# PaddleCV-SIG/MedicalSeg

Hardware: AMD Instinct MI355X
Metric: 3D-voxels/sec fwd+bwd, VNet 128^3 fp32 (higher is better)
Workload: dtype f32

## Files before the change

### medicalseg_amd/csrc/msk_conv_wbf.hip

```cpp
#include <type_traits>
#include "msk_wbf.h"
#ifndef WBF_TIN_SYNC
#define WBF_TIN_SYNC 1
#endif

#ifndef WBF_PROBE
#define WBF_PROBE 0
#endif
typedef _Float16 f16x8 __attribute__((ext_vector_type(8)));
typedef _Float16 f16x2 __attribute__((ext_vector_type(2)));

namespace {

constexpr int nxi_of(int K) { return K == 5 ? 8 : 6; }

__device__ __forceinline__ void split3_one(float x, unsigned short& hi, unsigned short& mid, unsigned short& lo) {
  hi = __builtin_bit_cast(unsigned short, (__bf16)x);
  const float r = x - __uint_as_float((unsigned)hi << 16);
  mid = __builtin_bit_cast(unsigned short, (__bf16)r);
  const float r2 = r - __uint_as_float((unsigned)mid << 16);
  lo = __builtin_bit_cast(unsigned short, (__bf16)r2);
}
__device__ __forceinline__ unsigned pack_f16_pair(float a, float b) {
  f32x2 v = {a, b};
// ... 533 lines not shown
  float4 win[WIN][2];
  const int t0 = blockIdx.z * a.t_per, t1 = min(a.T, t0 + a.t_per);
#pragma unroll
  for (int j = 0; j < WIN; ++j) dy_at(4 * t0 + j - PADW, win[j][0], win[j][1]);
  for (int t = t0; t < t1; ++t) {
#if WBF_TIN_SYNC
    __builtin_amdgcn_s_barrier();
#endif
    float4 nxt[4][2];
#pragma unroll
    for (int j = 0; j < 4; ++j) {
      const int w = 4 * (t + 1) + KEEP - PADW + j;
      if (t + 1 < t1) dy_at(w, nxt[j][0], nxt[j][1]);
      else nxt[j][0] = nxt[j][1] = z4;
    }
    float v[8][8];
    if (WV) {
#pragma unroll
      for (int q = 0; q < 2; ++q) {
        float wx[8], wy[8], wz[8], ww[8];
#pragma unroll
        for (int j = 0; j < 8; ++j) {
          const float4 e = j < WIN ? win[j < WIN ? j : 0][q] : z4;
          wx[j] = e.x; wy[j] = e.y; wz[j] = e.z; ww[j] = e.w;
        }
        tin_transform<0, K>(wx, v[q * 4 + 0]);
        tin_transform<0, K>(wy, v[q * 4 + 1]);
        tin_transform<0, K>(wz, v[q * 4 + 2]);
        tin_transform<0, K>(ww, v[q * 4 + 3]);
      }
#pragma unroll
      for (int xi = 0; xi < NXI; ++xi) store_xi<K, NP>(vb + t * tstep + (long)xi * a.v_xi, plane, v, xi, sc2);
    }
    if (WY) {
#pragma unroll
      for (int q = 0; q < 2; ++q) {
        float wx[8], wy[8], wz[8], ww[8];
#pragma unroll
        for (int j = 0; j < 4; ++j) {
          const float4 e = win[PADW + j][q];
          wx[j] = e.x; wy[j] = e.y; wz[j] = e.z; ww[j] = e.w;
        }
#pragma unroll
        for (int j = 4; j < 8; ++j) wx[j] = wy[j] = wz[j] = ww[j] = 0.f;
        tin_transform<1, K>(wx, v[q * 4 + 0]);
        tin_transform<1, K>(wy, v[q * 4 + 1]);
        tin_transform<1, K>(wz, v[q * 4 + 2]);
        tin_transform<1, K>(ww, v[q * 4 + 3]);
      }
#pragma unroll
      for (int xi = 0; xi < NXI; ++xi) store_xi<K, NP>(yb2 + t * tstep + (long)xi * b.y_xi, plane, v, xi, sc2);
    }
#pragma unroll
    for (int j = 0; j < KEEP; ++j) {
      win[j][0] = win[j + 4][0];
      win[j][1] = win[j + 4][1];
    }
#pragma unroll
    for (int j = 0; j < 4; ++j) {
      win[KEEP + j][0] = nxt[j][0];
      win[KEEP + j][1] = nxt[j][1];
    }
  }
  }
  if (want_cmax) wbf_cmax_commit(b.y_cmax, cg, cmx, true);
}

struct GemmArgs {
  const char* V;
  const char* U;
  float* M;
  int N, T, KC, CN, LD, LH, DP, HP;
  int tiles_d, tiles_h, ngrp, ksplit, kc_per;
  int tpb, nblk;
  long v_xi, v_plane;
  long u_xi;
  long m_xi;
};

__device__ __forceinline__ uint4 buf_load16(__amdgpu_buffer_rsrc_t r, unsigned lane_bytes, unsigned uniform_bytes) {
  return __builtin_bit_cast(uint4, __builtin_amdgcn_raw_buffer_load_b128(r, (int)lane_bytes, (int)uniform_bytes, 0));
}

typedef int i32x4 __attribute__((ext_vector_type(4)));
__device__ __forceinline__ void wbf_dma16(i32x4 rs, unsigned lds_addr, unsigned voff, unsigned soff) {
  asm volatile("s_mov_b32 m0, %0\n\ts_nop 0\n\tbuffer_load_dwordx4 %1, %2, %3 offen lds" ::"s"(lds_addr), "v"(voff), "s"(rs), "s"(soff) : "memory");
}

#define WBF_MFMA(acc, av, bv) \
  acc = __builtin_amdgcn_mfma_f32_32x32x16_bf16(__builtin_bit_cast(bf16x8, av), __builtin_bit_cast(bf16x8, bv), acc, 0, 0, 0)
#define WBF_MFMA_H(acc, av, bv) \
  acc = __builtin_amdgcn_mfma_f32_32x32x16_f16(__builtin_bit_cast(f16x8, av), __builtin_bit_cast(f16x8, bv), acc, 0, 0, 0)

template <int TH>
__device__ __forceinline__ void frag_pos(int r, int& a, int& b) {
  if (TH == 16) {
    if (r < 4) { a = 0; b = r; }
    else if (r < 12) { a = 0; b = r + 4; }
    else if (r < 16) { a = 0; b = r - 8; }
    else if (r < 20) { a = 1; b = r - 4; }
    else if (r < 28) { a = 1; b = r - 16; }
    else { a = 1; b = r - 28; }
  } else if (TH == 8) {
    if (r < 4) { a = 0; b = r; }
    else if (r < 12) { a = 1; b = r - 4; }
    else if (r < 16) { a = 0; b = r - 8; }
    else if (r < 20) { a = 3; b = r - 16; }
    else if (r < 28) { a = 2; b = r - 20; }
    else { a = 3; b = r - 24; }
  } else {
    a = r / TH;
    b = r % TH;
  }
}

template <int MR, int WM, int WN, int TD, int TH, int K, int NP, int BPF = 1>
__global__ void __launch_bounds__(WM * WN * 64)
wbf_gemm_k(GemmArgs a) {
  static_assert((WM * WN == 4 || WM * WN == 2) && WM * MR * 32 == TD * TH, "tile shape");
  constexpr int NT = WM * WN * 64;
  constexpr int NXI = nxi_of(K), T2 = K * K, PADK = (K - 1) / 2;
  constexpr int HDt = TD + K - 1, HPt = TH + K - 1, NSLOT = HDt * HPt, NPL = 2 * NP, NIT = NPL * NSLOT, ROUNDS = (NIT + NT - 1) / NT;
  __shared__ uint4 lds[ROUNDS * NT];

  const int tid = threadIdx.x;
  const int wave = __builtin_amdgcn_readfirstlane(tid >> 6), lane = tid & 63, li = lane & 31, lh = lane >> 5;
  const int wm = wave / WN, wn = wave % WN;

#pragma unroll 1
  for (int rep = 0; rep < a.tpb; ++rep) {
  int b = blockIdx.x + rep * gridDim.x;
  if (b >= a.nblk) break;
  if (rep > 0) __syncthreads();
  const int xi = b % NXI;
  b /= NXI;
  const int grp = b % a.ngrp;
  b /= a.ngrp;
  const int thi = b % a.tiles_h;
  b /= a.tiles_h;
  const int tdi = b % a.tiles_d;
  b /= a.tiles_d;
  const int t = b % a.T;
  b /= a.T;
  const int n = b % a.N;
  const int ks = b / a.N;

  unsigned voff[ROUNDS];
#pragma unroll
  for (int r = 0; r < ROUNDS; ++r) {
    int it = r * NT + tid;
    if (it >= NIT) it = 0;
    const int pk = it / NSLOT, slot = it - pk * NSLOT;
    const int row = slot / HPt, col = slot - row * HPt;
    voff[r] = (unsigned)(pk * a.v_plane + ((long)row * a.HP + col) * 16);
  }
  const char* vtile = a.V + (long)xi * a.v_xi + ((long)(n * a.T + t) * a.KC) * NPL * a.v_plane +
                      ((long)(tdi * TD + 2 - PADK) * a.HP + thi * TH + 2 - PADK) * 16;
  const __amdgpu_buffer_rsrc_t vres = __builtin_amdgcn_make_buffer_rsrc((void*)vtile, 0, 0xFFFFFFF0u, 0x00020000);
  const __amdgpu_buffer_rsrc_t ures =
      __builtin_amdgcn_make_buffer_rsrc((void*)(a.U + (long)xi * a.u_xi), 0, 0xFFFFFFF0u, 0x00020000);
  const unsigned ulane = (unsigned)(lh * a.CN + (grp * WN + wn) * 32 + li) * 16u;
  const unsigned ustep = (unsigned)a.CN * 32u;
  const unsigned uchunk = (unsigned)NP * ustep;
  const unsigned utap = (unsigned)a.KC * uchunk;

  int arow[MR];
#pragma unroll
  for (int mr = 0; mr < MR; ++mr) {
    int fa, fb;
    frag_pos<TH>(li, fa, fb);
// ... 140 lines not shown
  if (xi == 0) { c1 = c2 = c3 = 0.f; return; }
  if (xi == last) { c1 = c2 = 0.f; c3 = 1.f; return; }
  const float sg = (xi & 1) ? 1.f : -1.f;
  const int pr = (xi - 1) >> 1;
  const float p = pr == 0 ? 1.f : (pr == 1 ? 2.f : 0.5f);
  c1 = sg * p;
  c2 = p * p;
  c3 = sg * p * p * p;
}

#ifndef WBF_FUSED_BPF
#define WBF_FUSED_BPF 3
#endif
template <int MR, int WM, int WN, int TD, int TH, int K, int NP, bool STATS, int BPF = (NP == 2 ? WBF_FUSED_BPF : 1), int BL = 0>
__global__ void __launch_bounds__(WM * WN * 64, 2)
wbf_gemm_fused_k(FusedArgs f) {
  static_assert(WM * WN == 4 && WM * MR * 32 == TD * TH, "tile shape");
  const GemmArgs& a = f.g;
  constexpr int NT = WM * WN * 64;
  constexpr int NXI = nxi_of(K), T2 = K * K, PADK = (K - 1) / 2;
  constexpr int HDt = TD + K - 1, HPt = TH + K - 1, NSLOT = HDt * HPt, NPL = 2 * NP, NIT = NPL * NSLOT, ROUNDS = (NIT + NT - 1) / NT;
  constexpr int NBF = T2 * NP;
  constexpr int BROUNDS = (NBF + WM * WN - 1) / (WM * WN);
  static_assert(BL == 0 || NIT % 64 == 0, "weights through LDS: wave-granular tile");
  static_assert(BL != 1 || WN == 1, "B through LDS, whole stage: one column fragment");
  constexpr int PH = WN == 1 ? 4 : 5;
  constexpr int PQ_T[6] = {0, T2 * 1 / PH, T2 * 2 / PH, T2 * 3 / PH, PH > 4 ? T2 * 4 / PH : T2, T2};
  constexpr int PQ_FR = (T2 - PQ_T[PH - 1]) * NP * WN;
  constexpr int PQ_SLOT = PQ_FR * 64;
  static_assert(BL != 2 || (NP == 2 && WM * WN == 4 && WN <= 2 && PQ_T[1] * NP * WN >= 4), "pipelined form: fp16 x 2 pieces, four wavefronts");
  __shared__ uint4 lds[BL == 2 ? 2 * NIT + 2 * PQ_SLOT : (BL ? NIT + NBF * 64 : ROUNDS * NT)];

  const int tid = threadIdx.x;
  const int wave = __builtin_amdgcn_readfirstlane(tid >> 6), lane = tid & 63, li = lane & 31, lh = lane >> 5;
  const int wm = wave / WN, wn = wave % WN;

  int b = (blockIdx.x & 7) * f.per_xcd + (blockIdx.x >> 3);
  if ((int)(blockIdx.x >> 3) >= f.per_xcd || b >= a.nblk) return;
  const int tile_id = b;
  const int thi = b % a.tiles_h;
  b /= a.tiles_h;
  const int tdi = b % a.tiles_d;
  b /= a.tiles_d;
  const int t = b % a.T;
  const int n = b / a.T;

  unsigned voff[ROUNDS];
#pragma unroll
  for (int r = 0; r < ROUNDS; ++r) {
    int it = r * NT + tid;
    if (it >= NIT) it = 0;
    const int pk = it / NSLOT, slot = it - pk * NSLOT;
    const int row = slot / HPt, col = slot - row * HPt;
    voff[r] = (unsigned)(pk * a.v_plane + ((long)row * a.HP + col) * 16);
  }
  const char* vtile0 = a.V + ((long)(n * a.T + t) * a.KC) * NPL * a.v_plane +
                       ((long)(tdi * TD + 2 - PADK) * a.HP + thi * TH + 2 - PADK) * 16;
  const unsigned ulane = (unsigned)(lh * a.CN + wn * 32 + li) * 16u;
  const unsigned ustep = (unsigned)a.CN * 32u;
  const unsigned uchunk = (unsigned)NP * ustep;
  const unsigned utap = (unsigned)a.KC * uchunk;

  int arow[MR];
#pragma unroll
  for (int mr = 0; mr < MR; ++mr) {
    int fa, fb;
    frag_pos<TH>(li, fa, fb);
    arow[mr] = lh * NSLOT + ((wm * MR + mr) * (32 / TH) + fa) * HPt + fb;
  }

  f32x16 yo[4][MR];
#pragma unroll
  for (int i = 0; i < 4; ++i)
#pragma unroll
    for (int mr = 0; mr < MR; ++mr)
#pragma unroll
      for (int j = 0; j < 16; ++j) yo[i][mr][j] = 0.f;

  if constexpr (BL == 2) {
    const unsigned lds0 = (unsigned)(unsigned long)(__attribute__((address_space(3))) void*)lds;
    const int NS = NXI * a.KC;
    const unsigned voff_last = (ROUNDS - 1) * NT + wave * 64 < NIT ? voff[ROUNDS - 1] : voff[ROUNDS - 2];
    const int r_last = (ROUNDS - 1) * NT + wave * 64 < NIT ? ROUNDS - 1 : ROUNDS - 2;
    auto rsrc_of = [](const char* p_) {
      const unsigned long pa = (unsigned long)p_;
      i32x4 r_ = {(int)__builtin_amdgcn_readfirstlane((unsigned)pa), (int)(__builtin_amdgcn_readfirstlane((unsigned)(pa >> 32)) & 0xffffu),
                  (int)0xFFFFFFF0u, 0x00020000};
      return r_;
    };
    auto fill_tile = [&](int s_) {
      const int xi_ = s_ / a.KC, kc_ = s_ - xi_ * a.KC;
      const i32x4 vr = rsrc_of(vtile0 + (long)xi_ * a.v_xi);
      const unsigned so = (unsigned)(kc_ * NPL * a.v_plane);
      const unsigned dst = lds0 + (unsigned)((s_ & 1) * NIT + wave * 64) * 16u;
#pragma unroll
      for (int r = 0; r < ROUNDS - 1; ++r) wbf_dma16(vr, dst + (unsigned)(r * NT) * 16u, voff[r], so);
      wbf_dma16(vr, dst + (unsigned)(r_last * NT) * 16u, voff_last, so);
    };
    auto fill_weights = [&](int s_, auto qc) {
      constexpr int q = decltype(qc)::value;
      constexpr int f0 = PQ_T[q] * NP * WN, nf = (PQ_T[q + 1] - PQ_T[q]) * NP * WN, rounds = (nf + 3) / 4;
      const int xi_ = s_ / a.KC, kc_ = s_ - xi_ * a.KC;
      const i32x4 ur = rsrc_of(a.U + (long)xi_ * a.u_xi);
      const unsigned ukc = (unsigned)kc_ * uchunk;
#pragma unroll
      for (int r = 0; r < rounds; ++r) {
        int fr = r * 4 + wave;
        if (fr >= nf) fr -= 4;
        const int fg = (f0 + fr) / WN, fw = (f0 + fr) % WN;
        wbf_dma16(ur, lds0 + (unsigned)(2 * NIT + ((q + (s_ & PH & 1)) & 1) * PQ_SLOT + fr * 64) * 16u, (unsigned)(lh * a.CN + fw * 32 + li) * 16u,
                  (unsigned)(fg / NP) * utap + ukc + (unsigned)(fg % NP) * ustep);
      }
    };
    f32x16 acc[MR];
    int abase[MR];
    auto run_phase = [&](int s_, auto qc) {
      constexpr int q = decltype(qc)::value;
      constexpr int T0 = PQ_T[q], T1 = PQ_T[q + 1];
      const bool more = s_ + 1 < NS;
      if (q == 1 && more) asm volatile("s_waitcnt vmcnt(%0)" ::"n"(ROUNDS) : "memory");
      else asm volatile("s_waitcnt vmcnt(0)" ::: "memory");
      __builtin_amdgcn_s_barrier();
      asm volatile("" ::: "memory");
      if constexpr (q < PH - 1) fill_weights(s_, std::integral_constant<int, q + 1>{});
      else if (more) fill_weights(s_ + 1, std::integral_constant<int, 0>{});
      if (q == 0 && more) fill_tile(s_ + 1);
      const uint4* bl = lds + 2 * NIT + ((q + (s_ & PH & 1)) & 1) * PQ_SLOT + wn * 64 + lane;
      uint4 aq[2][MR][NP], bq[2][NP];
#pragma unroll
      for (int p = 0; p < NP; ++p) bq[T0 & 1][p] = bl[p * WN * 64];
#pragma unroll
      for (int mr = 0; mr < MR; ++mr) {
        const uint4* ap = lds + abase[mr] + (T0 / K) * HPt + (T0 % K);
#pragma unroll
        for (int p = 0; p < NP; ++p) aq[T0 & 1][mr][p] = ap[p * 2 * NSLOT];
      }
#pragma unroll
      for (int tap = T0; tap < T1; ++tap) {
        const int cur = tap & 1, nx = cur ^ 1;
        if (tap + 1 < T1) {
#pragma unroll
          for (int p = 0; p < NP; ++p) bq[nx][p] = bl[((tap + 1 - T0) * NP + p) * WN * 64];
#pragma unroll
          for (int mr = 0; mr < MR; ++mr) {
            const uint4* ap = lds + abase[mr] + ((tap + 1) / K) * HPt + ((tap + 1) % K);
#pragma unroll
            for (int p = 0; p < NP; ++p) aq[nx][mr][p] = ap[p * 2 * NSLOT];
          }
        }
        __builtin_amdgcn_sched_barrier(0);
        const uint4 bdown = wbf_hi_down(bq[cur][0]);
#pragma unroll
        for (int mr = 0; mr < MR; ++mr) WBF_MFMA_H(acc[mr], aq[cur][mr][NP - 1], bdown);
#pragma unroll
        for (int mr = 0; mr < MR; ++mr) WBF_MFMA_H(acc[mr], aq[cur][mr][0], bq[cur][NP - 1]);
#pragma unroll
        for (int mr = 0; mr < MR; ++mr) WBF_MFMA_H(acc[mr], aq[cur][mr][0], bq[cur][0]);
        __builtin_amdgcn_sched_barrier(0);
      }
    };
    fill_weights(0, std::integral_constant<int, 0>{});
    fill_tile(0);
#pragma unroll 1
    for (int s_ = 0; s_ < NS; ++s_) {
      const int xi = s_ / a.KC, kc = s_ - xi * a.KC;
      if (kc == 0) {
#pragma unroll
        for (int mr = 0; mr < MR; ++mr)
#pragma unroll
          for (int j = 0; j < 16; ++j) acc[mr][j] = 0.f;
      }
#pragma unroll
// ... 1080 lines not shown
```

### medicalseg_amd/csrc/msk_wbf.h

```cpp
#pragma once
#include "msk_conv.h"

typedef __bf16 bf16x8 __attribute__((ext_vector_type(8)));
typedef __bf16 bf16x2 __attribute__((ext_vector_type(2)));
typedef float f32x16 __attribute__((ext_vector_type(16)));
typedef float f32x4 __attribute__((ext_vector_type(4)));
typedef float f32x2 __attribute__((ext_vector_type(2)));

__device__ __forceinline__ void wbf_split3_pair(float x0, float x1, unsigned& hi, unsigned& mid, unsigned& lo) {
  f32x2 x = {x0, x1};
  hi = __builtin_bit_cast(unsigned, __builtin_convertvector(x, bf16x2));
  f32x2 r = {x0 - __uint_as_float(hi << 16), x1 - __uint_as_float(hi & 0xffff0000u)};
  mid = __builtin_bit_cast(unsigned, __builtin_convertvector(r, bf16x2));
  f32x2 r2 = {r.x - __uint_as_float(mid << 16), r.y - __uint_as_float(mid & 0xffff0000u)};
  lo = __builtin_bit_cast(unsigned, __builtin_convertvector(r2, bf16x2));
}

typedef _Float16 wbf_f16x2 __attribute__((ext_vector_type(2)));
__device__ __forceinline__ void wbf_split2h_pair(float x0, float x1, unsigned& hi, unsigned& lo) {
  f32x2 x = {x0, x1};
  const wbf_f16x2 h = __builtin_convertvector(x, wbf_f16x2);
  hi = __builtin_bit_cast(unsigned, h);
  const f32x2 hf = __builtin_convertvector(h, f32x2);
  f32x2 r = {x0 - hf.x, x1 - hf.y};
  lo = __builtin_bit_cast(unsigned, __builtin_convertvector(r, wbf_f16x2));
}
constexpr float kWbfLoScale = 2048.f;
__device__ __forceinline__ void wbf_split2hs_pair(float x0, float x1, unsigned& hi, unsigned& lo) {
  f32x2 x = {x0, x1};
  const wbf_f16x2 h = __builtin_convertvector(x, wbf_f16x2);
  hi = __builtin_bit_cast(unsigned, h);
  const f32x2 hf = __builtin_convertvector(h, f32x2);
  f32x2 r = {(x0 - hf.x) * kWbfLoScale, (x1 - hf.y) * kWbfLoScale};
  lo = __builtin_bit_cast(unsigned, __builtin_convertvector(r, wbf_f16x2));
}
typedef _Float16 wbf_f16x8 __attribute__((ext_vector_type(8)));
__device__ __forceinline__ uint4 wbf_hi_down(uint4 h) {
  const wbf_f16x8 v = __builtin_bit_cast(wbf_f16x8, h) * (_Float16)(1.0f / kWbfLoScale);
  return __builtin_bit_cast(uint4, v);
}
constexpr int kWbfXformHeader = 512;
constexpr int kWbfAmaxWays = 64;
__device__ __forceinline__ float wbf_amax_of(const float* amax) {
  const float4* p = reinterpret_cast<const float4*>(amax);
  float m = 0.f;
#pragma unroll
  for (int i = 0; i < kWbfAmaxWays / 4; ++i) {
    const float4 q = p[i];
    m = fmaxf(fmaxf(m, fmaxf(q.x, q.y)), fmaxf(q.z, q.w));
  }
  return m;
}
__device__ __forceinline__ float wbf_scale_from(float a) {
  if (!(a > 0.f) || !(a < 3.0e38f)) return 1.f;
  int e;
  (void)frexpf(a, &e);
  return ldexpf(1.f, 10 - e);
}
__device__ __forceinline__ float wbf_scale_of(const float* amax) {
  if (!amax) return 1.f;
  return wbf_scale_from(wbf_amax_of(amax));
}

struct WbfTinArgs {
  const float* src;
  int sld;
  long svn;
  int svd, svh, svw;
  int N, LD, LH, LW, T, CK, KC;
  int DP, HP;
  char* V;
  long v_xi;
  int lane_map;
  const float* amax;
  float* amax_copy;
  int t_per;
  int c_real;
  float* cmax;
};
__device__ __forceinline__ int wbf_chan_shift(float tensor_amax, float chan_max) {
  if (!(chan_max > 0.f) || !(tensor_amax > 0.f) || !(tensor_amax < 3.0e38f)) return 0;
  int ea, ec;
  (void)frexpf(tensor_amax, &ea);
  (void)frexpf(chan_max, &ec);
  const int s = ea - ec;
  return s < 0 ? 0 : (s > 15 ? 15 : s);
}
#ifndef WBF_CMAX_PRECHECK
#define WBF_CMAX_PRECHECK 1
#endif
__device__ __forceinline__ void wbf_cmax_commit(float* cmax, int cg, float (&mx)[8], bool wave_cg) {
  unsigned* q = reinterpret_cast<unsigned*>(cmax) + cg * 8;
#if WBF_CMAX_PRECHECK
  const bool precheck = gridDim.x * gridDim.y * gridDim.z > 1024u;
  unsigned cur[8] = {0u, 0u, 0u, 0u, 0u, 0u, 0u, 0u};
  if (precheck) {
#pragma unroll
    for (int j = 0; j < 8; ++j) cur[j] = __hip_atomic_load(q + j, __ATOMIC_RELAXED, __HIP_MEMORY_SCOPE_AGENT);
  }
#endif
#pragma unroll
  for (int j = 0; j < 8; ++j) {
    float m = mx[j];
#pragma unroll
    for (int o = 32; o >= 4; o >>= 1) m = fmaxf(m, __shfl_xor(m, o, 64));
    if (wave_cg) {
      m = fmaxf(m, __shfl_xor(m, 2, 64));
      m = fmaxf(m, __shfl_xor(m, 1, 64));
    }
    mx[j] = m;
  }
  const int lane = threadIdx.x & 63;
  if (lane < (wave_cg ? 1 : 4)) {
#if WBF_CMAX_PRECHECK
#pragma unroll
    for (int j = 0; j < 8; ++j)
      if (mx[j] > 0.f && __float_as_uint(mx[j]) > cur[j]) atomicMax(q + j, __float_as_uint(mx[j]));
#else
#pragma unroll
    for (int j = 0; j < 8; ++j)
      if (mx[j] > 0.f) atomicMax(q + j, __float_as_uint(mx[j]));
#endif
  }
}
int msk_wbf_transform(msk_ctx* ctx, int mode, int K, int NP, const WbfTinArgs& a);

struct WbfBnBwd {
  const float* y;
  int yld;
  const float* dout;
  int dld;
  const float *scale, *shift, *alpha, *mean, *invstd, *sums;
  float invM;
  char* Y;
  const float* amax;
  long y_xi;
  const float* maxes;
  float* y_cmax;
  int coef_stride;
  int sums_stride;
  int res_is_input;
};
int msk_wbf_transform_dual(msk_ctx* ctx, int K, int NP, const WbfTinArgs& a, const WbfBnBwd& bn, bool write_v);
inline int wbf_pieces(const msk_ctx* ctx, int K) { return (K == 3 && ctx->conv_fp16) ? 1 : (ctx->conv_split == 2 ? 2 : 3); }
// ... 58 lines not shown
```

### medicalseg_amd/csrc/msk_wgrad_wbf.hip

```cpp
#include "msk_wbf.h"

typedef short s16x4 __attribute__((ext_vector_type(4)));
typedef short s16x8 __attribute__((ext_vector_type(8)));
typedef _Float16 f16x8 __attribute__((ext_vector_type(8)));

namespace {

struct WgArgs {
  const char* V;
  const char* Y;
  float* P;
  int N, T, KCA, KCB, DP, HP;
  int tiles_d, tiles_h, ntiles, ksplit, tiles_per;
  int ncob;
  long v_xi, y_xi, plane;
  const float *y_cmax, *y_amax;
};

__device__ __forceinline__ s16x4 tr_read(const char* lds_base, unsigned byte_off) {
  return __builtin_amdgcn_ds_read_tr16_b64_v4i16((__attribute__((address_space(3))) s16x4*)(lds_base + byte_off));
}

#define WGW_MFMA(acc, av, bv) \
  acc = __builtin_amdgcn_mfma_f32_16x16x32_bf16(__builtin_bit_cast(bf16x8, av), __builtin_bit_cast(bf16x8, bv), acc, 0, 0, 0)
#define WGW_MFMA_H(acc, av, bv) \
  acc = __builtin_amdgcn_mfma_f32_16x16x32_f16(__builtin_bit_cast(f16x8, av), __builtin_bit_cast(f16x8, bv), acc, 0, 0, 0)

constexpr int wg_nxi(int K) { return K == 5 ? 8 : 6; }

#ifndef WGW_LB
#define WGW_LB 3
#endif
#ifndef WGW_PIPE
#define WGW_PIPE 0
#endif
template <int TH, int K, int NP>
#if WGW_LB > 0
__global__ void __launch_bounds__(256, WGW_LB)
#else
__global__ void __launch_bounds__(256)
#endif
wbf_wgrad_k(WgArgs a) {
  constexpr int NXI = wg_nxi(K), T2 = K * K, PADK = (K - 1) / 2, NPL = 2 * NP;
  constexpr int NT0 = K == 5 ? 7 : 3, NT1 = K == 5 ? 6 : 2;
  constexpr int TD = 8, HPt = TH + K - 1, NSV = (TD + K - 1) * HPt, NSY = TD * TH;
  constexpr int RV1 = (NSV + 63) / 64, RY1 = (NSY + 63) / 64;
  constexpr int PSV = RV1 * 1024 + (TH == 16 ? 64 : 128);
  constexpr int PSY = RY1 * 1024 + 64;
  constexpr int YBASE = NPL * PSV;
  constexpr int NRV = NPL * RV1, NRY = 2 * NPL * RY1, NR = NRV + NRY, RPW = (NR + 3) / 4;
  constexpr int KSTEPS = TD * TH / 32, ROWS_PER_STEP = 32 / TH;
  __shared__ __attribute__((aligned(16))) char lds[NPL * PSV + 2 * NPL * PSY];

  const int tid = threadIdx.x;
  const int wave = __builtin_amdgcn_readfirstlane(tid >> 6), lane = tid & 63;
  const int g = lane >> 4, i = lane & 15;

  int b = blockIdx.x;
  const int xi = b % NXI;
  b /= NXI;
  const int cob = b % a.ncob;
  b /= a.ncob;
  const int kci = b % a.KCA;
  const int ks = b / a.KCA;

  const __amdgpu_buffer_rsrc_t vres =
      __builtin_amdgcn_make_buffer_rsrc((void*)(a.V + (long)xi * a.v_xi), 0, 0xFFFFFFF0u, 0x00020000);
  const __amdgpu_buffer_rsrc_t yres =
      __builtin_amdgcn_make_buffer_rsrc((void*)(a.Y + (long)xi * a.y_xi), 0, 0xFFFFFFF0u, 0x00020000);

  unsigned voff[RPW];
  int ldst[RPW];
#pragma unroll
  for (int j = 0; j < RPW; ++j) {
    const int R = wave + 4 * j;
    if (R < NRV) {
      const int pk = R / RV1, sub = R - pk * RV1;
      int slot = sub * 64 + lane;
      if (slot >= NSV) slot = 0;
      const int row = slot / HPt, col = slot - row * HPt;
      voff[j] = (unsigned)(((long)kci * NPL + pk) * a.plane + ((long)(row + 2 - PADK) * a.HP + col + 2 - PADK) * 16);
      ldst[j] = pk * PSV + sub * 1024;
    } else {
      const int Ry = R - NRV;
      const int cp = Ry / RY1, sub = Ry - cp * RY1;
      int slot = sub * 64 + lane;
      if (slot >= NSY) slot = 0;
      const int row = slot / TH, col = slot - row * TH;
      voff[j] = (unsigned)(((long)cob * 2 * NPL + cp) * a.plane + ((long)(row + 2) * a.HP + col + 2) * 16);
      ldst[j] = YBASE + cp * PSY + sub * 1024;
    }
  }

  const int q0 = 8 * g + (i >> 2);
  const int khalf = (i & 3) >> 1, sub8 = (i & 1) * 8;
  const unsigned va = (unsigned)(khalf * PSV + ((q0 / TH) * HPt + (q0 % TH)) * 16 + sub8);
  const int tap0 = wave == 0 ? 0 : NT0 - NT1 + NT1 * wave, ntap = wave == 0 ? NT0 : NT1;
  unsigned tapoff[NT0];
#pragma unroll
  for (int j = 0; j < NT0; ++j) {
    const int tp = min(tap0 + j, T2 - 1);
    tapoff[j] = (unsigned)(((tp / K) * HPt + (tp % K)) * 16);
  }
  const unsigned ya = (unsigned)(YBASE + khalf * PSY + ((q0 / TH) * TH + (q0 % TH)) * 16 + sub8);

  f32x4 acc[NT0][2];
#pragma unroll
  for (int j = 0; j < NT0; ++j)
#pragma unroll
    for (int c = 0; c < 2; ++c) acc[j][c] = (f32x4){0.f, 0.f, 0.f, 0.f};

  int shb[2] = {0, 0};
  if (NP == 2 && a.y_cmax && a.y_amax) {
    const float ya_max = wbf_amax_of(a.y_amax);
    shb[0] = wbf_chan_shift(ya_max, a.y_cmax[cob * 32 + i]);
    shb[1] = wbf_chan_shift(ya_max, a.y_cmax[cob * 32 + 16 + i]);
  }
  const _Float16 mb[2] = {(_Float16)ldexpf(1.f, shb[0]), (_Float16)ldexpf(1.f, shb[1])};
  const _Float16 mb_dn[2] = {(_Float16)ldexpf(1.f, shb[0] - 11), (_Float16)ldexpf(1.f, shb[1] - 11)};
  auto fmul = [](s16x8 v, _Float16 m) { return __builtin_bit_cast(s16x8, __builtin_bit_cast(f16x8, v) * m); };

  const int t0 = ks * a.tiles_per;
  const int t1 = min(a.ntiles, t0 + a.tiles_per);
  const int tiles_nt = a.tiles_d * a.tiles_h;
  for (int tile = t0; tile < t1; ++tile) {
    const int nt = tile / tiles_nt, rem = tile - nt * tiles_nt;
    const int tdi = rem / a.tiles_h, thi = rem - tdi * a.tiles_h;
    const unsigned origin = (unsigned)(((long)(tdi * TD) * a.HP + thi * TH) * 16);
    const unsigned vso = (unsigned)((long)nt * a.KCA * NPL * a.plane) + origin;
    const unsigned yso = (unsigned)((long)nt * a.KCB * NPL * a.plane) + origin;
    __syncthreads();
#pragma unroll
    for (int j = 0; j < RPW; ++j) {
      const int R = wave + 4 * j;
      if (R < NRV)
        __builtin_amdgcn_raw_ptr_buffer_load_lds(vres, (__attribute__((address_space(3))) void*)(lds + ldst[j]), 16,
                                                 (int)voff[j], (int)vso, 0, 0);
      else if (R < NR)
        __builtin_amdgcn_raw_ptr_buffer_load_lds(yres, (__attribute__((address_space(3))) void*)(lds + ldst[j]), 16,
                                                 (int)voff[j], (int)yso, 0, 0);
    }
    asm volatile("s_waitcnt vmcnt(0)" ::: "memory");
    __syncthreads();

    auto load_b = [&](int kst, s16x8 (&bq0)[2], s16x8 (&bq1)[2], s16x8 (&bq2)[2], s16x8 (&bdh)[2], s16x8 (&bdl)[2]) {
#pragma unroll
      for (int c = 0; c < 2; ++c) {
        s16x8 t[NP];
#pragma unroll
        for (int p = 0; p < NP; ++p) {
          const unsigned o = ya + (unsigned)((c * NPL + p * 2) * PSY + kst * ROWS_PER_STEP * TH * 16);
          const s16x4 lo4 = tr_read(lds, o), hi4 = tr_read(lds, o + 64);
          t[p] = __builtin_shufflevector(lo4, hi4, 0, 1, 2, 3, 4, 5, 6, 7);
        }
        bq0[c] = t[0]; bq1[c] = t[NP / 2]; bq2[c] = t[NP - 1];
        bdh[c] = t[0]; bdl[c] = t[0];
        if (NP == 2) {
          bdh[c] = fmul(t[0], mb_dn[c]);
          bdl[c] = fmul(t[NP - 1], mb_dn[c]);
          bq0[c] = fmul(t[0], mb[c]);
        }
      }
    };
#if WGW_PIPE
    s16x8 nb0[2], nb1[2], nb2[2], nbh[2], nbl[2];
    load_b(0, nb0, nb1, nb2, nbh, nbl);
#endif
#pragma unroll
    for (int kst = 0; kst < KSTEPS; ++kst) {
      s16x8 bq[2][3], bdh[2], bdl[2];
#if WGW_PIPE
#pragma unroll
      for (int c = 0; c < 2; ++c) { bq[c][0] = nb0[c]; bq[c][1] = nb1[c]; bq[c][2] = nb2[c]; bdh[c] = nbh[c]; bdl[c] = nbl[c]; }
      if (kst + 1 < KSTEPS) load_b(kst + 1, nb0, nb1, nb2, nbh, nbl);
#else
      {
        s16x8 t0[2], t1[2], t2[2];
        load_b(kst, t0, t1, t2, bdh, bdl);
#pragma unroll
        for (int c = 0; c < 2; ++c) { bq[c][0] = t0[c]; bq[c][1] = t1[c]; bq[c][2] = t2[c]; }
      }
#endif
#pragma unroll
      for (int j = 0; j < NT0; ++j) {
        if (j < ntap) {
          s16x8 aq[NP];
          const unsigned vt = va + tapoff[j];
#pragma unroll
          for (int p = 0; p < NP; ++p) {
            const unsigned o = vt + (unsigned)(p * 2 * PSV + kst * ROWS_PER_STEP * HPt * 16);
            const s16x4 lo4 = tr_read(lds, o), hi4 = tr_read(lds, o + 64);
            aq[p] = __builtin_shufflevector(lo4, hi4, 0, 1, 2, 3, 4, 5, 6, 7);
          }
#pragma unroll
          for (int c = 0; c < 2; ++c) {
            if (NP == 3) {
              WGW_MFMA(acc[j][c], aq[NP - 1], bq[c][0]);
              WGW_MFMA(acc[j][c], aq[0], bq[c][2]);
              WGW_MFMA(acc[j][c], aq[NP / 2], bq[c][1]);
              WGW_MFMA(acc[j][c], aq[NP / 2], bq[c][0]);
              WGW_MFMA(acc[j][c], aq[0], bq[c][1]);
              WGW_MFMA(acc[j][c], aq[0], bq[c][0]);
            } else if (NP == 2) {
              WGW_MFMA_H(acc[j][c], aq[NP - 1], bdh[c]);
              WGW_MFMA_H(acc[j][c], aq[0], bdl[c]);
              WGW_MFMA_H(acc[j][c], aq[0], bq[c][0]);
            } else {
              WGW_MFMA_H(acc[j][c], aq[0], bq[c][0]);
            }
          }
        }
      }
    }
  }

  float* pb = a.P + (((((long)xi * a.ksplit + ks) * a.KCA + kci) * a.ncob + cob) * T2 + tap0) * 512;
  const float undo[2] = {ldexpf(1.f, -shb[0]), ldexpf(1.f, -shb[1])};
#pragma unroll
  for (int j = 0; j < NT0; ++j)
    if (j < ntap) {
#pragma unroll
      for (int c = 0; c < 2; ++c)
#pragma unroll
        for (int r = 0; r < 4; ++r) pb[j * 512 + (4 * g + r) * 32 + c * 16 + i] = acc[j][c][r] * undo[c];
    }
}

template <int K>
__global__ void __launch_bounds__(256)
wbf_wgrad_reduce_k(const float* __restrict__ P, int ksplit, int NS, int KCA, int ncob, int CA, int CB, int tsd, int tsh,
                   int tsw, float* __restrict__ dw, int accumulate, const float* __restrict__ y_amax,
                   const float* __restrict__ v_amax, int scaled) {
  constexpr int NXI = wg_nxi(K), T2 = K * K, T3 = K * K * K;
  const double G5[8][5] = {{-1, 0, 0, 0, 0},
                           {-2.0 / 9, -2.0 / 9, -2.0 / 9, -2.0 / 9, -2.0 / 9},
                           {-2.0 / 9, 2.0 / 9, -2.0 / 9, 2.0 / 9, -2.0 / 9},
                           {1.0 / 90, 1.0 / 45, 2.0 / 45, 4.0 / 45, 8.0 / 45},
                           {1.0 / 90, -1.0 / 45, 2.0 / 45, -4.0 / 45, 8.0 / 45},
                           {32.0 / 45, 16.0 / 45, 8.0 / 45, 4.0 / 45, 2.0 / 45},
                           {32.0 / 45, -16.0 / 45, 8.0 / 45, -4.0 / 45, 2.0 / 45},
                           {0, 0, 0, 0, 1}};
  const double G3[6][3] = {{0.25, 0, 0},           {-1.0 / 6, -1.0 / 6, -1.0 / 6}, {-1.0 / 6, 1.0 / 6, -1.0 / 6},
                           {1.0 / 24, 1.0 / 12, 1.0 / 6}, {1.0 / 24, -1.0 / 12, 1.0 / 6},  {0, 0, 1}};
  __shared__ double sh[8][8][32];
  const double oscale = scaled ? 1.0 / ((double)wbf_scale_of(y_amax) * (double)wbf_scale_of(v_amax)) : 1.0;
  const int lane = threadIdx.x & 31, w8 = threadIdx.x >> 5, slice = w8 % NS, sub = w8 / NS, SUB = 8 / NS;
  const long groups = (long)T2 * CA * ncob;
  const long slab = (long)KCA * ncob * T2 * 512;
  const long rounds = (groups + SUB - 1) / SUB;
  for (long ri = blockIdx.x; ri < rounds; ri += gridDim.x) {
    const long gi = ri * SUB + sub;
    const bool live = gi < groups;
    const int cob = (int)(gi % ncob);
    long r_ = gi / ncob;
    const int ca = (int)(r_ % CA);
    const int row = (int)(r_ / CA);
    const long off = ((((long)(ca >> 4) * ncob + cob) * T2 + row) * 16 + (ca & 15)) * 32 + lane;
    {
      double acc[NXI];
#pragma unroll
      for (int xi = 0; xi < NXI; ++xi) acc[xi] = 0.0;
      if (live) {
        const float* p = P + off;
        const long xstep = (long)ksplit * slab;
        for (int z = slice; z < ksplit; z += NS) {
          float v[NXI];
#pragma unroll
          for (int xi = 0; xi < NXI; ++xi) v[xi] = p[(long)xi * xstep + (long)z * slab];
#pragma unroll
          for (int xi = 0; xi < NXI; ++xi) acc[xi] += (double)v[xi];
        }
      }
#pragma unroll
      for (int xi = 0; xi < NXI; ++xi) sh[w8][xi][lane] = acc[xi];
    }
    __syncthreads();
    if (slice == 0 && live) {
      double s[NXI];
#pragma unroll
      for (int xi = 0; xi < NXI; ++xi) {
        double t = sh[w8][xi][lane];
        for (int k = 1; k < NS; ++k) t += sh[w8 + k][xi][lane];
        s[xi] = t;
      }
      const int cb = cob * 32 + lane;
      float* o = dw + ((long)cb * CA + ca) * T3 + (row / K) * tsd + (row % K) * tsh;
#pragma unroll
      for (int kw = 0; kw < K; ++kw) {
        double v = 0.0;
#pragma unroll
        for (int xi = 0; xi < NXI; ++xi) v += (K == 5 ? G5[xi][kw] : G3[xi][kw]) * s[xi];
        v *= oscale;
        float* q = o + kw * tsw;
        *q = accumulate ? *q + (float)v : (float)v;
      }
    }
    __syncthreads();
  }
}

template <int K>
__global__ void __launch_bounds__(256)
wbf_wgrad_reduce_rows_k(const float* __restrict__ P, int ksplit, int KCA, int ncob, int CA, int CB, int tsd, int tsh, int tsw,
                        float* __restrict__ dw, int accumulate, const float* __restrict__ y_amax, const float* __restrict__ v_amax,
                        int scaled) {
  constexpr int NXI = wg_nxi(K), T2 = K * K, T3 = K * K * K, PITCH = T3 + 4;
  const double G5[8][5] = {{-1, 0, 0, 0, 0},
                           {-2.0 / 9, -2.0 / 9, -2.0 / 9, -2.0 / 9, -2.0 / 9},
                           {-2.0 / 9, 2.0 / 9, -2.0 / 9, 2.0 / 9, -2.0 / 9},
                           {1.0 / 90, 1.0 / 45, 2.0 / 45, 4.0 / 45, 8.0 / 45},
                           {1.0 / 90, -1.0 / 45, 2.0 / 45, -4.0 / 45, 8.0 / 45},
                           {32.0 / 45, 16.0 / 45, 8.0 / 45, 4.0 / 45, 2.0 / 45},
                           {32.0 / 45, -16.0 / 45, 8.0 / 45, -4.0 / 45, 2.0 / 45},
                           {0, 0, 0, 0, 1}};
  const double G3[6][3] = {{0.25, 0, 0},           {-1.0 / 6, -1.0 / 6, -1.0 / 6}, {-1.0 / 6, 1.0 / 6, -1.0 / 6},
                           {1.0 / 24, 1.0 / 12, 1.0 / 6}, {1.0 / 24, -1.0 / 12, 1.0 / 6},  {0, 0, 1}};
  __shared__ float tile[32 * PITCH];
  const double oscale = scaled ? 1.0 / ((double)wbf_scale_of(y_amax) * (double)wbf_scale_of(v_amax)) : 1.0;
  const int lane = threadIdx.x & 31, w8 = threadIdx.x >> 5;
  const int cob = blockIdx.x % ncob, ca = blockIdx.x / ncob;
  const long slab = (long)KCA * ncob * T2 * 512;
  const long xstep = (long)ksplit * slab;
  for (int row = w8; row < T2; row += 8) {
    const float* p = P + ((((long)(ca >> 4) * ncob + cob) * T2 + row) * 16 + (ca & 15)) * 32 + lane;
    double acc[NXI];
#pragma unroll
    for (int xi = 0; xi < NXI; ++xi) acc[xi] = 0.0;
    for (int z = 0; z < ksplit; ++z) {
      float v[NXI];
#pragma unroll
      for (int xi = 0; xi < NXI; ++xi) v[xi] = p[(long)xi * xstep + (long)z * slab];
#pragma unroll
      for (int xi = 0; xi < NXI; ++xi) acc[xi] += (double)v[xi];
    }
    float* o = tile + lane * PITCH + (row / K) * tsd + (row % K) * tsh;
#pragma unroll
    for (int kw = 0; kw < K; ++kw) {
      double v = 0.0;
#pragma unroll
      for (int xi = 0; xi < NXI; ++xi) v += (K == 5 ? G5[xi][kw] : G3[xi][kw]) * acc[xi];
      o[kw * tsw] = (float)(v * oscale);
    }
  }
  __syncthreads();
  float* base = dw + ((long)cob * 32 * CA + ca) * T3;
  for (int i = threadIdx.x; i < 32 * T3; i += 256) {
    const int cb = i / T3, tap = i - cb * T3;
    float* q = base + (long)cb * CA * T3 + tap;
    const float v = tile[cb * PITCH + tap];
    *q = accumulate ? *q + v : v;
  }
}

}

namespace {
template <int K, int NP>
int run_wgrad_pipeline(msk_ctx* ctx, const WGrad& g, const WbfGeom& geo, bool shared_geom, int TH) {
  constexpr int NXI = wg_nxi(K), T2 = K * K, NPL = 2 * NP;
  const int* pm = geo.perm;
  const int LD = geo.LD, LH = geo.LH, LW = geo.LW;
  const int vstr[3] = {g.BH * g.BW, g.BW, 1};
  const int tstr[3] = {K * K, K, 1};
  const int T = geo.T, KCA = g.CA / 16, KCB = g.CB / 16, ncob = g.CB / 32;
  const int tiles_d = (LD + 7) / 8, tiles_h = (LH + TH - 1) / TH;
  const int DP = geo.DP, HP = geo.HP;
  const long ntiles = (long)g.N * T * tiles_d * tiles_h;
  if (ntiles > 0x7fffffffL) return 0;

  const long base_blocks = (long)NXI * KCA * ncob;
  const long per_cu = ctx->wgrad_wino_rounds > 0 ? ctx->wgrad_wino_rounds : 3;
  long ksplit = (per_cu * ctx->num_cu + base_blocks / 2) / base_blocks;
  if (ksplit < 1) ksplit = 1;
  if (ksplit > ntiles) ksplit = ntiles;
  const int tiles_per = (int)((ntiles + ksplit - 1) / ksplit);
  ksplit = (ntiles + tiles_per - 1) / tiles_per;

  const size_t plane = (size_t)DP * HP * 16;
  const size_t v_xi = (size_t)g.N * T * KCA * NPL * plane, y_xi = (size_t)g.N * T * KCB * NPL * plane;
  if (v_xi >= 0xFFFFFFF0ull || y_xi >= 0xFFFFFFF0ull) return 0;
  const size_t p_floats = (size_t)NXI * ksplit * KCA * ncob * T2 * 512;
  const size_t vb = (NXI * v_xi + 255) & ~(size_t)255, yb = (NXI * y_xi + 255) & ~(size_t)255;
  const bool have_v = g.xform != nullptr && shared_geom &&
                      msk_wbf_xform_bytes(g.N, g.AD, g.AH, g.AW, g.CA, g.CB, K, NP) == NXI * v_xi + kWbfXformHeader;
  const bool have_y = g.yform != nullptr;
  if ((have_y || g.yfuse) && !(have_v && shared_geom)) return 0;
  char* wsp = (char*)msk_workspace(ctx, (have_v ? 0 : vb) + (have_y ? 0 : yb) + p_floats * sizeof(float) + 256);
  if (!wsp) return -1;
  char* V = have_v ? (char*)const_cast<void*>(g.xform) + kWbfXformHeader : wsp;
  const float* v_amax = nullptr;
  if (NP != 3 && have_v) v_amax = (const float*)g.xform;
  char* Y = have_y ? (char*)const_cast<void*>(g.yform) : (have_v ? wsp : wsp + vb);
  float* P = (float*)(have_y ? (have_v ? wsp : wsp + vb) : Y + yb);

  WbfTinArgs ta{};
  ta.src = g.A; ta.sld = g.ald;
  ta.svn = (long)g.BD * g.BH * g.BW; ta.svd = vstr[pm[0]]; ta.svh = vstr[pm[1]]; ta.svw = vstr[pm[2]];
  ta.N = g.N; ta.LD = LD; ta.LH = LH; ta.LW = LW; ta.T = T; ta.CK = g.CA; ta.KC = KCA;
  ta.DP = DP; ta.HP = HP; ta.V = V; ta.v_xi = (long)v_xi;
  const float* y_cmax = nullptr;
  const int cmax_slots_b = (g.CB + kWbfAmaxWays - 1) / kWbfAmaxWays;
  if (!have_v) {
    if (NP != 3) {
      v_amax = g.a_amax ? g.a_amax : msk_absmax(ctx, g.A, g.ald, g.CA, (long)g.N * g.AD * g.AH * g.AW);
      if (!v_amax) return -1;
      ta.amax = v_amax;
    }
    if (msk_wbf_transform(ctx, 0, K, NP, ta) != 0) return -1;
  }
  ta.src = g.B; ta.sld = g.bld; ta.CK = g.CB; ta.KC = KCB; ta.V = Y; ta.v_xi = (long)y_xi;
  const float* y_amax = nullptr;
  if (g.yfuse) {
    WbfBnBwd bn = *g.yfuse;
    bn.Y = Y;
    bn.y_xi = (long)y_xi;
    y_amax = bn.amax;
    if (NP == 2) {
      bn.y_cmax = msk_scalar_slots(ctx, cmax_slots_b);
      if (!bn.y_cmax) return -1;
      y_cmax = bn.y_cmax;
    }
    if (msk_wbf_transform_dual(ctx, K, NP, ta, bn, false) != 0) return -1;
  } else if (have_y) {
    y_amax = g.y_amax;
    y_cmax = NP == 2 ? g.y_cmax : nullptr;
  } else {
    if (NP != 3) {
      y_amax = g.b_amax ? g.b_amax : msk_absmax(ctx, g.B, g.bld, g.cb_real > 0 ? g.cb_real : g.CB, (long)g.N * g.BD * g.BH * g.BW);
      if (!y_amax) return -1;
    }
    ta.amax = y_amax;
    ta.c_real = g.cb_real;
    if (NP == 2) {
      ta.cmax = msk_scalar_slots(ctx, cmax_slots_b);
      if (!ta.cmax) return -1;
      y_cmax = ta.cmax;
    }
    if (msk_wbf_transform(ctx, 1, K, NP, ta) != 0) return -1;
  }

  WgArgs wa{};
  wa.V = V; wa.Y = Y; wa.P = P;
  wa.N = g.N; wa.T = T; wa.KCA = KCA; wa.KCB = KCB; wa.DP = DP; wa.HP = HP;
  wa.tiles_d = tiles_d; wa.tiles_h = tiles_h; wa.ntiles = (int)ntiles; wa.ksplit = (int)ksplit; wa.tiles_per = tiles_per;
  wa.ncob = ncob; wa.v_xi = (long)v_xi; wa.y_xi = (long)y_xi; wa.plane = (long)plane;
  if (NP == 2 && ctx->wgrad_renorm) { wa.y_cmax = y_cmax; wa.y_amax = y_amax; }
  const long nblk = base_blocks * ksplit;
  {
    const char* tag = NP == 3 ? "wbf_wgrad_k" : (NP == 2 ? "wbf_wgrad_h2_k" : "wbf_wgrad_f16_k");
    if (ctx->prof && ctx->prof_shapes) {
      char buf[200];
      snprintf(buf, sizeof(buf), "%s[ca=%d,cb=%d,n=%d,dhw=%dx%dx%d,k=%d,ks=%ld]", tag, g.CA, g.CB, g.N, g.BD, g.BH, g.BW, K, ksplit);
      tag = msk_intern_tag(ctx, buf);
    }
// ... 92 lines not shown
```

Measured before the change: 237.7 million.

## Double-buffer V tiles in wgrad kernel to overlap DMA with MFMA

```diff
diff --git a/medicalseg_amd/csrc/msk_conv_wbf.hip b/medicalseg_amd/csrc/msk_conv_wbf.hip
--- a/medicalseg_amd/csrc/msk_conv_wbf.hip
+++ b/medicalseg_amd/csrc/msk_conv_wbf.hip
@@ -639,10 +639,6 @@
   return __builtin_bit_cast(uint4, __builtin_amdgcn_raw_buffer_load_b128(r, (int)lane_bytes, (int)uniform_bytes, 0));
 }
 
-typedef int i32x4 __attribute__((ext_vector_type(4)));
-__device__ __forceinline__ void wbf_dma16(i32x4 rs, unsigned lds_addr, unsigned voff, unsigned soff) {
-  asm volatile("s_mov_b32 m0, %0\n\ts_nop 0\n\tbuffer_load_dwordx4 %1, %2, %3 offen lds" ::"s"(lds_addr), "v"(voff), "s"(rs), "s"(soff) : "memory");
-}
 
 #define WBF_MFMA(acc, av, bv) \
   acc = __builtin_amdgcn_mfma_f32_32x32x16_bf16(__builtin_bit_cast(bf16x8, av), __builtin_bit_cast(bf16x8, bv), acc, 0, 0, 0)
@@ -949,12 +945,7 @@
     const int NS = NXI * a.KC;
     const unsigned voff_last = (ROUNDS - 1) * NT + wave * 64 < NIT ? voff[ROUNDS - 1] : voff[ROUNDS - 2];
     const int r_last = (ROUNDS - 1) * NT + wave * 64 < NIT ? ROUNDS - 1 : ROUNDS - 2;
-    auto rsrc_of = [](const char* p_) {
-      const unsigned long pa = (unsigned long)p_;
-      i32x4 r_ = {(int)__builtin_amdgcn_readfirstlane((unsigned)pa), (int)(__builtin_amdgcn_readfirstlane((unsigned)(pa >> 32)) & 0xffffu),
-                  (int)0xFFFFFFF0u, 0x00020000};
-      return r_;
-    };
+    auto rsrc_of = [](const char* p_) { return wbf_rsrc(p_); };
     auto fill_tile = [&](int s_) {
       const int xi_ = s_ / a.KC, kc_ = s_ - xi_ * a.KC;
       const i32x4 vr = rsrc_of(vtile0 + (long)xi_ * a.v_xi);
diff --git a/medicalseg_amd/csrc/msk_wbf.h b/medicalseg_amd/csrc/msk_wbf.h
--- a/medicalseg_amd/csrc/msk_wbf.h
+++ b/medicalseg_amd/csrc/msk_wbf.h
@@ -60,6 +60,21 @@
 __device__ __forceinline__ float wbf_scale_of(const float* amax) {
   if (!amax) return 1.f;
   return wbf_scale_from(wbf_amax_of(amax));
+}
+
+typedef int i32x4 __attribute__((ext_vector_type(4)));
+#pragma clang diagnostic push
+#pragma clang diagnostic ignored "-Winline-asm"
+__device__ __forceinline__ void wbf_dma16(i32x4 rs, unsigned lds_addr, unsigned voff, unsigned soff) {
+  asm volatile("s_mov_b32 m0, %0\n\ts_nop 0\n\tbuffer_load_dwordx4 %1, %2, %3 offen lds" ::"s"(lds_addr), "v"(voff), "s"(rs), "s"(soff)
+               : "memory", "m0");
+}
+#pragma clang diagnostic pop
+__device__ __forceinline__ i32x4 wbf_rsrc(const void* p) {
+  const unsigned long pa = (unsigned long)p;
+  i32x4 r = {(int)__builtin_amdgcn_readfirstlane((unsigned)pa), (int)(__builtin_amdgcn_readfirstlane((unsigned)(pa >> 32)) & 0xffffu),
+             (int)0xFFFFFFF0u, 0x00020000};
+  return r;
 }
 
 struct WbfTinArgs {
diff --git a/medicalseg_amd/csrc/msk_wgrad_wbf.hip b/medicalseg_amd/csrc/msk_wgrad_wbf.hip
--- a/medicalseg_amd/csrc/msk_wgrad_wbf.hip
+++ b/medicalseg_amd/csrc/msk_wgrad_wbf.hip
@@ -28,29 +28,30 @@
 
 constexpr int wg_nxi(int K) { return K == 5 ? 8 : 6; }
 
-#ifndef WGW_LB
-#define WGW_LB 3
-#endif
-#ifndef WGW_PIPE
-#define WGW_PIPE 0
-#endif
+constexpr int wg_rounds(int slots) { return (slots + 63) / 64; }
+constexpr int wg_psv(int TH, int K) { return wg_rounds((8 + K - 1) * (TH + K - 1)) * 1024 + (TH == 16 ? 64 : 128); }
+constexpr int wg_psy(int TH) { return wg_rounds(8 * TH) * 1024 + 64; }
+constexpr int wg_vimg(int TH, int K, int NP) { return 2 * NP * wg_psv(TH, K); }
+constexpr int wg_yimg(int TH, int NP) { return 2 * 2 * NP * wg_psy(TH); }
+constexpr bool wg_dbv(int TH, int K, int NP) { return K == 5 && NP == 2 && 3 * (2 * wg_vimg(TH, K, NP) + wg_yimg(TH, NP)) <= 160 * 1024; }
+constexpr int wg_lds_bytes(int TH, int K, int NP) { return (wg_dbv(TH, K, NP) ? 2 : 1) * wg_vimg(TH, K, NP) + wg_yimg(TH, NP); }
+constexpr int wg_wgs_per_cu(int TH, int K, int NP) { return 160 * 1024 / wg_lds_bytes(TH, K, NP) < 3 ? 160 * 1024 / wg_lds_bytes(TH, K, NP) : 3; }
+
 template <int TH, int K, int NP>
-#if WGW_LB > 0
-__global__ void __launch_bounds__(256, WGW_LB)
-#else
-__global__ void __launch_bounds__(256)
-#endif
+__global__ void __launch_bounds__(256, wg_wgs_per_cu(TH, K, NP))
 wbf_wgrad_k(WgArgs a) {
   constexpr int NXI = wg_nxi(K), T2 = K * K, PADK = (K - 1) / 2, NPL = 2 * NP;
   constexpr int NT0 = K == 5 ? 7 : 3, NT1 = K == 5 ? 6 : 2;
   constexpr int TD = 8, HPt = TH + K - 1, NSV = (TD + K - 1) * HPt, NSY = TD * TH;
-  constexpr int RV1 = (NSV + 63) / 64, RY1 = (NSY + 63) / 64;
-  constexpr int PSV = RV1 * 1024 + (TH == 16 ? 64 : 128);
-  constexpr int PSY = RY1 * 1024 + 64;
-  constexpr int YBASE = NPL * PSV;
+  constexpr int RV1 = wg_rounds(NSV), RY1 = wg_rounds(NSY);
+  constexpr int PSV = wg_psv(TH, K);
+  constexpr int PSY = wg_psy(TH);
+  constexpr int VIMG = wg_vimg(TH, K, NP);
+  constexpr bool DBV = wg_dbv(TH, K, NP);
+  constexpr int YBASE = (DBV ? 2 : 1) * VIMG;
   constexpr int NRV = NPL * RV1, NRY = 2 * NPL * RY1, NR = NRV + NRY, RPW = (NR + 3) / 4;
   constexpr int KSTEPS = TD * TH / 32, ROWS_PER_STEP = 32 / TH;
-  __shared__ __attribute__((aligned(16))) char lds[NPL * PSV + 2 * NPL * PSY];
+  __shared__ __attribute__((aligned(16))) char lds[wg_lds_bytes(TH, K, NP)];
 
   const int tid = threadIdx.x;
   const int wave = __builtin_amdgcn_readfirstlane(tid >> 6), lane = tid & 63;
@@ -64,10 +65,8 @@
   const int kci = b % a.KCA;
   const int ks = b / a.KCA;
 
-  const __amdgpu_buffer_rsrc_t vres =
-      __builtin_amdgcn_make_buffer_rsrc((void*)(a.V + (long)xi * a.v_xi), 0, 0xFFFFFFF0u, 0x00020000);
-  const __amdgpu_buffer_rsrc_t yres =
-      __builtin_amdgcn_make_buffer_rsrc((void*)(a.Y + (long)xi * a.y_xi), 0, 0xFFFFFFF0u, 0x00020000);
+  const i32x4 vres = wbf_rsrc(a.V + (long)xi * a.v_xi), yres = wbf_rsrc(a.Y + (long)xi * a.y_xi);
+  const unsigned lds0 = (unsigned)(unsigned long)(__attribute__((address_space(3))) void*)lds;
 
   unsigned voff[RPW];
   int ldst[RPW];
@@ -123,25 +122,27 @@
   const int t0 = ks * a.tiles_per;
   const int t1 = min(a.ntiles, t0 + a.tiles_per);
   const int tiles_nt = a.tiles_d * a.tiles_h;
-  for (int tile = t0; tile < t1; ++tile) {
+  auto fill = [&](int tile, unsigned vimg, bool do_v, bool do_y) {
     const int nt = tile / tiles_nt, rem = tile - nt * tiles_nt;
     const int tdi = rem / a.tiles_h, thi = rem - tdi * a.tiles_h;
     const unsigned origin = (unsigned)(((long)(tdi * TD) * a.HP + thi * TH) * 16);
     const unsigned vso = (unsigned)((long)nt * a.KCA * NPL * a.plane) + origin;
     const unsigned yso = (unsigned)((long)nt * a.KCB * NPL * a.plane) + origin;
-    __syncthreads();
 #pragma unroll
     for (int j = 0; j < RPW; ++j) {
       const int R = wave + 4 * j;
-      if (R < NRV)
-        __builtin_amdgcn_raw_ptr_buffer_load_lds(vres, (__attribute__((address_space(3))) void*)(lds + ldst[j]), 16,
-                                                 (int)voff[j], (int)vso, 0, 0);
-      else if (R < NR)
-        __builtin_amdgcn_raw_ptr_buffer_load_lds(yres, (__attribute__((address_space(3))) void*)(lds + ldst[j]), 16,
-                                                 (int)voff[j], (int)yso, 0, 0);
-    }
-    asm volatile("s_waitcnt vmcnt(0)" ::: "memory");
-    __syncthreads();
+      const bool is_v = 4 * j + 3 < NRV || (4 * j < NRV && R < NRV), live = 4 * j + 3 < NR || (4 * j < NR && R < NR);
+      if (is_v) { if (do_v) wbf_dma16(vres, lds0 + vimg + (unsigned)ldst[j], voff[j], vso); }
+      else if (live && do_y) wbf_dma16(yres, lds0 + (unsigned)ldst[j], voff[j], yso);
+    }
+  };
+  if (t0 < t1) fill(t0, 0u, true, true);
+  for (int tile = t0; tile < t1; ++tile) {
+    const unsigned curv = DBV ? (unsigned)((tile - t0) & 1) * VIMG : 0u;
+    asm volatile("s_waitcnt vmcnt(0) lgkmcnt(0)" ::: "memory");
+    __builtin_amdgcn_s_barrier();
+    asm volatile("" ::: "memory");
+    if (DBV && tile + 1 < t1) fill(tile + 1, VIMG - curv, true, false);
 
     auto load_b = [&](int kst, s16x8 (&bq0)[2], s16x8 (&bq1)[2], s16x8 (&bq2)[2], s16x8 (&bdh)[2], s16x8 (&bdl)[2]) {
 #pragma unroll
@@ -162,30 +163,20 @@
         }
       }
     };
-#if WGW_PIPE
-    s16x8 nb0[2], nb1[2], nb2[2], nbh[2], nbl[2];
-    load_b(0, nb0, nb1, nb2, nbh, nbl);
-#endif
 #pragma unroll
     for (int kst = 0; kst < KSTEPS; ++kst) {
       s16x8 bq[2][3], bdh[2], bdl[2];
-#if WGW_PIPE
-#pragma unroll
-      for (int c = 0; c < 2; ++c) { bq[c][0] = nb0[c]; bq[c][1] = nb1[c]; bq[c][2] = nb2[c]; bdh[c] = nbh[c]; bdl[c] = nbl[c]; }
-      if (kst + 1 < KSTEPS) load_b(kst + 1, nb0, nb1, nb2, nbh, nbl);
-#else
       {
         s16x8 t0[2], t1[2], t2[2];
         load_b(kst, t0, t1, t2, bdh, bdl);
 #pragma unroll
         for (int c = 0; c < 2; ++c) { bq[c][0] = t0[c]; bq[c][1] = t1[c]; bq[c][2] = t2[c]; }
       }
-#endif
 #pragma unroll
       for (int j = 0; j < NT0; ++j) {
         if (j < ntap) {
           s16x8 aq[NP];
-          const unsigned vt = va + tapoff[j];
+          const unsigned vt = curv + va + tapoff[j];
 #pragma unroll
           for (int p = 0; p < NP; ++p) {
             const unsigned o = vt + (unsigned)(p * 2 * PSV + kst * ROWS_PER_STEP * HPt * 16);
@@ -211,6 +202,12 @@
           }
         }
       }
+    }
+    if (tile + 1 < t1) {
+      asm volatile("s_waitcnt lgkmcnt(0)" ::: "memory");
+      __builtin_amdgcn_s_barrier();
+      asm volatile("" ::: "memory");
+      fill(tile + 1, 0u, !DBV, true);
     }
   }
 
@@ -369,7 +366,8 @@
   if (ntiles > 0x7fffffffL) return 0;
 
   const long base_blocks = (long)NXI * KCA * ncob;
-  const long per_cu = ctx->wgrad_wino_rounds > 0 ? ctx->wgrad_wino_rounds : 3;
+  const long per_cu = ctx->wgrad_wino_rounds > 0 ? ctx->wgrad_wino_rounds
+                                                 : (TH == 16 ? wg_wgs_per_cu(16, K, NP) : wg_wgs_per_cu(8, K, NP));
   long ksplit = (per_cu * ctx->num_cu + base_blocks / 2) / base_blocks;
   if (ksplit < 1) ksplit = 1;
   if (ksplit > ntiles) ksplit = ntiles;
```

Measured after the change: 237.8 million, median of 5. No clear change (+0.0%).
